# sjz5202/DisenLink

Hardware: AMD Instinct MI355X
Metric: edges/sec (aggregate+score) at K=8 d=64 (higher is better)
Workload: dtype f32; 1 GPU; squirrel_real (edge list of the parity fixture)(seed 0): N=5201, edge rows=217073, 85/5/10 split, E_sym=342129, scored train pairs P=1009603 (m=5), K=8, d=64, beta=0.5, t=1.0; forward route+aggregate+score_pairs; K=8, d=64, n_nodes=5201, E_sym=342129, P=1009603

## Files before the change

### disenlink_amd/_lib.py

```python
from __future__ import annotations

import ctypes as C
import os

PKG = os.path.dirname(os.path.abspath(__file__))
LIB_PATH = os.path.join(PKG, "libdisenlink_hip.so")


class DlCsrPlan(C.Structure):
    _fields_ = [
        ("n_rows", C.c_int32), ("row_offset", C.c_int32), ("n_total", C.c_int32), ("n_entries", C.c_int32),
        ("rowptr", C.c_void_p), ("col", C.c_void_p),
        ("seg_len", C.c_int32), ("n_seg", C.c_int32),
        ("seg_row", C.c_void_p), ("seg_beg", C.c_void_p), ("seg_end", C.c_void_p), ("seg_slot", C.c_void_p),
        ("n_slices", C.c_int32), ("slice_max_seg", C.c_int32), ("slice_seg0", C.c_void_p),
        ("n_multi", C.c_int32), ("n_slots", C.c_int32), ("multi_row", C.c_void_p), ("multi_slot0", C.c_void_p),
        ("slot_multi", C.c_void_p), ("unit_count", C.c_void_p),
    ]


class DlGraph(C.Structure):
    _fields_ = [("csr", DlCsrPlan), ("route", DlCsrPlan), ("rev", C.c_void_p), ("route_mirror", C.c_int32)]


class DlPairHub(C.Structure):
    _fields_ = [("n_blocks", C.c_int32), ("block_row", C.c_void_p),
                ("n_items", C.c_int32), ("n_slices", C.c_int32), ("slice_max_item", C.c_int32),
                ("slice_item0", C.c_void_p), ("item_block", C.c_void_p), ("item_step", C.c_void_p),
                ("n_steps", C.c_int32), ("step_v", C.c_void_p), ("step_u", C.c_void_p), ("step_q", C.c_void_p),
                ("step_q2", C.c_void_p), ("n_entries", C.c_int32),
                ("rest", DlCsrPlan), ("rest_pair", C.c_void_p), ("rest_pair2", C.c_void_p)]


class DlPairIncidence(C.Structure):
    _fields_ = [("csr", DlCsrPlan), ("inc_pair", C.c_void_p), ("n_pairs", C.c_int32), ("entry_yw", C.c_void_p),
                ("inc_pair2", C.c_void_p), ("n_second", C.c_int32), ("hub", C.POINTER(DlPairHub))]


class DlHostCsr(C.Structure):
    _fields_ = [("n_nodes", C.c_int32), ("n_entries", C.c_int32), ("rowptr", C.POINTER(C.c_int32)),
                ("col", C.POINTER(C.c_int32)), ("rev", C.POINTER(C.c_int32))]


class DlHostPlan(C.Structure):
    _fields_ = [(n, C.c_int32) for n in ("seg_len", "n_seg", "n_slices", "slice_max_seg", "n_multi", "n_slots")] + \
               [(n, C.POINTER(C.c_int32)) for n in ("seg_row", "seg_beg", "seg_end", "seg_slot", "slice_seg0",
# ... 301 lines not shown
```

### disenlink_amd/csrc/dl_api.hip

```cpp
#include <stdarg.h>
#include <string.h>
#include "dl_common.h"
#include "dl_kernels.h"

namespace dl {

static thread_local char g_err[512] = "";
static int g_force_generic = 0;

void set_error(const char* fmt, ...) {
    va_list ap;
    va_start(ap, fmt);
    vsnprintf(g_err, sizeof(g_err), fmt, ap);
    va_end(ap);
}

int check_launch(const char* what) {
    hipError_t e = hipGetLastError();
    if (e != hipSuccess) {
        set_error("%s: %s", what, hipGetErrorString(e));
        return DL_E_LAUNCH;
    }
    return DL_OK;
}
// ... 202 lines not shown
    if (int rc = check_dtype(c, K, d, dtype)) return rc;
    DL_REQUIRE(t != 0.0f, "temperature is 0");
    if (c->n_rows == 0) return DL_OK;
    DL_REQUIRE(Z && s, "Z or s is NULL");
    if (c->n_entries > 0) DL_REQUIRE(p && a, "p or a is NULL");
    if (use_fast(c, K, d, dtype)) {
        Workspace w;
        if (int rc = check_workspace(c, K, d, ws, ws_bytes, &w)) return rc;
        const dl_csr_plan* rp = &g->route;
        const bool have = has_seg_plan(rp) && rp->n_rows == c->n_rows && rp->n_total == c->n_total &&
                          rp->row_offset == c->row_offset && rp->rowptr == c->rowptr && rp->col == c->col;
        const bool mirror = have && g->route_mirror != 0;
        if (mirror)
            DL_REQUIRE((g->rev != nullptr || c->n_entries == 0) && c->row_offset == 0 && c->n_rows == c->n_total,
                       "route_mirror needs rev and an unsharded plan");
        return fast_route_fwd(c, have ? rp : nullptr, mirror, g->rev, Z, K, d, dtype, t, p, a, s, w.vec_part,
                              (hipStream_t)stream);
    }
    return generic_route_fwd(c, (const float*)Z, K, d, t, p, a, s, (hipStream_t)stream);
}

int dl_aggregate_fwd(const dl_graph* g, const void* Z, int K, int d, dl_dtype dtype, float beta, const uint8_t* p,
                     const float* a, const float* s, void* H, void* ws, size_t ws_bytes, void* stream) {
    DL_REQUIRE(g != nullptr, "graph is NULL");
    const dl_csr_plan* c = &g->csr;
    if (int rc = check_plan(c, "graph")) return rc;
    if (int rc = check_shape(K, d)) return rc;
    if (int rc = check_dtype(c, K, d, dtype)) return rc;
    if (c->n_rows == 0) return DL_OK;
    DL_REQUIRE(Z && s && H, "Z, s or H is NULL");
    if (c->n_entries > 0) DL_REQUIRE(p && a, "p or a is NULL");
// ... 878 lines not shown
```

### disenlink_amd/csrc/dl_config.h

```cpp
#pragma once

namespace dl {

struct Config {
    int stream_rows;
    bool fwd_group_kernel;
    bool fwd_hub;
    int auc_target;
    bool project_fp32_mfma;
    int fwd_groups;
    long long fwd_block_rows;
    long long bwd_block_bytes;
    int bwd_target;
    int inkernel_combine;
    int rank_slices;
    int mine_tiles;
    int sparse_seg;
};

const Config& config();
void config_reload();

}
```

### disenlink_amd/csrc/dl_config.hip

```cpp
#include <stdlib.h>
#include <algorithm>
#include <mutex>
#include "dl_config.h"
#include "disenlink_hip.h"

namespace dl {
namespace {

Config g_config;
std::once_flag g_once;

bool flag(const char* name) {
    const char* e = getenv(name);
    return e != nullptr && e[0] != '\0' && !(e[0] == '0' && e[1] == '\0');
}
long long number(const char* name) {
    const char* e = getenv(name);
    return e != nullptr && e[0] != '\0' ? atoll(e) : 0;
}

void read_environment() {
    Config c;
    const char* sr = getenv("DL_STREAM_ROWS");
    c.stream_rows = (sr == nullptr || sr[0] == '\0') ? -1 : (sr[0] == '1' ? 1 : 0);
    c.fwd_group_kernel = flag("DL_FWD_GROUP_KERNEL");
    const char* fh = getenv("DL_FWD_HUB");
    c.fwd_hub = !(fh != nullptr && fh[0] == '0' && fh[1] == '\0');
    c.auc_target = (int)std::max(0LL, number("DL_AUC_TARGET"));
    c.project_fp32_mfma = getenv("DL_PROJECT_FP32_MFMA") != nullptr;
    c.fwd_groups = (int)std::max(0LL, number("DL_FWD_GROUPS"));
    c.fwd_block_rows = std::max(0LL, number("DL_FWD_BLOCK_ROWS"));
    c.bwd_block_bytes = std::max(0LL, number("DL_BWD_BLOCK_BYTES"));
    c.bwd_target = (int)std::max(0LL, number("DL_BWD_TARGET"));
    const char* ic = getenv("DL_INKERNEL_COMBINE");
    c.inkernel_combine = (ic == nullptr || ic[0] == '\0') ? 1 : std::max(0, std::min(2, atoi(ic)));
    c.rank_slices = (int)std::max(0LL, number("DL_RANK_SLICES"));
    c.mine_tiles = (int)std::max(0LL, std::min(1LL << 20, number("DL_MINE_TILES")));
    c.sparse_seg = (int)std::max(0LL, std::min(1LL << 20, number("DL_SPARSE_SEG")));
    g_config = c;
}

}
// ... 15 lines not shown
```

### disenlink_amd/csrc/dl_fast.h

```cpp
#pragma once
#include <stdlib.h>
#include <type_traits>
#include "dl_common.h"
#include "dl_kernels.h"

namespace dl {
namespace fast {

typedef unsigned short bf16_t;

template <int VEC>
struct Chunk {
    float v[VEC];
};

__device__ __forceinline__ float bf16_to_f32(unsigned int hi16) { return __uint_as_float(hi16 << 16); }
__device__ __forceinline__ unsigned int f32_to_bf16(float f) {
    unsigned int u = __float_as_uint(f);
    if ((u & 0x7fffffffu) > 0x7f800000u) return (u >> 16) | 0x40u;
    return (u + 0x7fffu + ((u >> 16) & 1u)) >> 16;
}

template <typename T>
struct Tab;
// ... 139 lines not shown
typedef float v2f __attribute__((ext_vector_type(2)));
__device__ __forceinline__ float dot4_packed(const float4& a, const float4& b) {
    const v2f a0 = {a.x, a.y}, a1 = {a.z, a.w}, b0 = {b.x, b.y}, b1 = {b.z, b.w};
    const v2f p = __builtin_elementwise_fma(a1, b1, a0 * b0);
    return p.x + p.y;
}

template <typename V>
__device__ __forceinline__ const __attribute__((address_space(1))) V* uniform_row(const void* table, size_t byte_off) {
    const __attribute__((address_space(1))) char* row =
        reinterpret_cast<const __attribute__((address_space(1))) char*>((const __attribute__((address_space(1))) void*)table) + byte_off;
    asm volatile("" : "+s"(row));
    return reinterpret_cast<const __attribute__((address_space(1))) V*>(row);
}
__device__ __forceinline__ float4 as_float4(dl_vf4 v) { return make_float4(v.x, v.y, v.z, v.w); }

template <int K, int D, int VEC>
__device__ __forceinline__ void stage_row(float* dst, const Chunk<VEC> (&acc)[K], int c) {
#pragma unroll
    for (int kk = 0; kk < K; ++kk) store_f32<VEC>(dst + kk * D + c * VEC, acc[kk]);
}

template <int K, int D, typename T, int NROWS, bool NO_GROUP_ROWS = false>
struct Stage {
    using GE = Geo<K, D, T>;
    static constexpr int VEC = GE::VEC, G = GE::G;
    static constexpr int NG = DL_WAVE / G;
    static constexpr int ROWF = NROWS * GE::ROW;
    static constexpr bool GROUPS_IN_LDS = !NO_GROUP_ROWS && NROWS == 2 && (size_t)WAVES_PER_BLOCK * NG * ROWF * sizeof(float) <= 64 * 1024;
    static constexpr int SG = GROUPS_IN_LDS ? NG : 1;
// ... 198 lines not shown
```

### disenlink_amd/csrc/dl_kernels.h

```cpp
#pragma once
#include <hip/hip_runtime.h>
#include "disenlink_hip.h"

namespace dl {

int generic_route_fwd(const dl_csr_plan* c, const float* Z, int K, int d, float t, uint8_t* p, float* a, float* s,
                      hipStream_t st);
int generic_aggregate_fwd(const dl_csr_plan* c, const float* Z, int K, int d, float beta, const uint8_t* p,
                          const float* a, const float* s, float* H, hipStream_t st);
int generic_score_pairs_fwd(const float* Z, const float* H, int K, int d, float t, const int32_t* pu,
                            const int32_t* pv, int P, float* prob, hipStream_t st);
int generic_score_pairs_bwd(const dl_pair_incidence* inc, const float* Z, const float* H, int K, int d, float t,
                            const float* prob, const float* g_prob, float* dZ, float* dH, hipStream_t st);
int generic_bwd_phase1(const dl_csr_plan* c, const float* Z, int K, int d, float beta, const uint8_t* p,
                       const float* a, const float* s, const float* dH, float* dw, float* dwr, float* ds,
                       hipStream_t st);
int generic_bwd_phase2(const dl_csr_plan* c, const float* Z, int K, int d, float beta, float t, const uint8_t* p,
                       const float* a, const float* s, const float* dH, const float* dw, const float* dwr,
                       const float* ds, const float* dz_in, const float* scale, float* dZ, hipStream_t st);

bool fast_supported(int K, int d, int dtype);
int fast_route_fwd(const dl_csr_plan* g, const dl_csr_plan* route, bool mirror, const int32_t* rev, const void* Z,
                   int K, int d, int dtype, float t, uint8_t* p, float* a, float* s, float* s_part, hipStream_t st);
int fast_aggregate_fwd(const dl_csr_plan* g, const void* Z, int K, int d, int dtype, float beta, const uint8_t* p,
                       const float* a, const float* s, void* H, float* h_part, hipStream_t st);
int fast_bwd_phase1(const dl_csr_plan* g, const void* Z, int K, int d, int dtype, float beta, const uint8_t* p,
                    const float* a, const float* s, const float* dH, float* dw, float* dwr, float* ds,
                    float* ds_part, hipStream_t st);
int fast_bwd_phase2(const dl_csr_plan* g, const void* Z, int K, int d, int dtype, float beta, float t,
                    const uint8_t* p, const float* a, const float* s, const float* dH, const float* dw,
                    const float* dwr, const float* ds, const float* dz_in, const float* scale, float* dZ, float* dz_part, hipStream_t st);
int fast_score_pairs_fwd(const dl_pair_incidence* by_u, const void* Z, const void* H, int K, int d, int dtype,
                         float t, float* prob, float* coef, hipStream_t st);
int fast_score_pairs_train(const dl_pair_incidence* inc, const void* Z, const void* H, int K, int d, int dtype, float t,
                           const float* y, const float* w, float* prob, float* dZ, float* dH, float* part, hipStream_t st);
int fast_score_pairs_bwd(const dl_pair_incidence* inc, const void* Z, const void* H, int K, int d, int dtype,
                         float t, const float* prob, const float* g_prob, const float* coef, float* dZ, float* dH,
                         float* part, hipStream_t st);
// ... 150 lines not shown
```

### disenlink_amd/csrc/dl_route.hip

```cpp
#include "dl_fast.h"

namespace dl {
namespace fast {

template <int K, int D, typename T, bool MIRROR>
__global__ __launch_bounds__(BLOCK, (K <= 8 && sizeof(T) == 4) ? 8 : (K <= 10 ? 6 : (K <= 16 ? 4 : 1))) void route_seg_kernel(dl_csr_plan g, const int32_t* __restrict__ rev,
                                                          const T* __restrict__ Z, float t,
                                                          uint8_t* __restrict__ p, float* __restrict__ a) {
    using GE = Geo<K, D, T>;
    using FL = typename GE::FL;
    constexpr int VEC = GE::VEC, G = GE::G, EPW = GE::EPW, KP = FL::KP, VPL = FL::VPL;
    const WaveSeg ws = load_wave_seg(g);
    if (!ws.active) return;
    const SegInfo si = ws.si;
    const int lane = lane_id();
    const int c = lane % G, grp = lane / G;
    const int kb = FL::factor_base(c);

    Chunk<VEC> zi[K];
#pragma unroll
    for (int k = 0; k < K; ++k) zi[k] = Tab<T>::load(Z + (size_t)si.grow * GE::ROW + k * D + c * VEC);

    int my_col = si.grow, my_rev = 0;
    if (si.beg + lane < si.end) {
// ... 15 lines not shown
        int win = 255;
#pragma unroll
        for (int i = 0; i < VPL; ++i) {
            const float al = ex[i] / S;
            if (kb + i < K && (win == 255 || beats(al, best))) { best = al; win = kb + i; }
        }
        group_argmax_first<G>(best, win);
        if (MIRROR) {
            const int r = entry_scalar<EPW>(my_rev, base - si.beg, grp);
            if (live && c == 0) { p[e] = (uint8_t)win; a[e] = best; }
            if (live && c == 1 % G && r != e) { p[r] = (uint8_t)win; a[r] = best; }
        } else {
            if (live && c == 0) { p[e] = (uint8_t)win; a[e] = best; }
        }
    }
}

constexpr int ROWSUM_SUB = 4;
constexpr int ROWSUM_POS_PER_BLOCK = BLOCK / ROWSUM_SUB;

template <int CTRL>
__device__ __forceinline__ float dpp_move(float v) {
    return __int_as_float(__builtin_amdgcn_update_dpp(0, __float_as_int(v), CTRL, 0xF, 0xF, true));
}
template <int CTRL>
__device__ __forceinline__ int dpp_move_i(int v) {
    return __builtin_amdgcn_update_dpp(-1, v, CTRL, 0xF, 0xF, false);
}

template <int KP>
// ... 107 lines not shown
    else if (K <= 8) hipLaunchKernelGGL(s_rowsum_thread_kernel<8>, grid, block, 0, st, *g, K, p, a, s, reg);
    else if (K <= 16) hipLaunchKernelGGL(s_rowsum_thread_kernel<16>, grid, block, 0, st, *g, K, p, a, s, reg);
    else hipLaunchKernelGGL(s_rowsum_thread_kernel<32>, grid, block, 0, st, *g, K, p, a, s, reg);
}

void launch_vec_combine(const dl_csr_plan* g, int K, const float* part, int mode, const float* s_raw,
                        float* out, hipStream_t st) {
    if (g->n_multi <= 0) return;
    hipLaunchKernelGGL(vec_combine_kernel, dim3(wave_blocks(g->n_multi)), dim3(BLOCK), 0, st, *g, K, pow2_at_least(K),
                       part, mode, s_raw, out);
}

template <int K, int D, typename T>
struct RouteOps {
    static int route_fwd(const dl_csr_plan* g, const dl_csr_plan* route, bool mirror, const int32_t* rev,
                         const void* Z, float t, uint8_t* p, float* a, float* s, float* s_part, hipStream_t st) {
        const dl_csr_plan* rp = route ? route : g;
        if (mirror)
            hipLaunchKernelGGL((route_seg_kernel<K, D, T, true>), dim3(seg_blocks(rp)), dim3(BLOCK), 0, st, *rp, rev,
                               (const T*)Z, t, p, a);
        else
            hipLaunchKernelGGL((route_seg_kernel<K, D, T, false>), dim3(seg_blocks(rp)), dim3(BLOCK), 0, st, *rp, rev,
                               (const T*)Z, t, p, a);
        (void)s_part;
        launch_s_rowsum(g, K, p, a, s, st);
        return check_launch("route_fwd(fast)");
    }
};

}

bool fast_supported(int K, int d, int dtype) {
#define X(KK, DD) if (K == KK && d == DD) return true;
    if (dtype == DL_F32) { DL_FAST_SHAPES_F32(X) }
    if (dtype == DL_BF16) { DL_FAST_SHAPES_BF16(X) }
#undef X
    return false;
}

int fast_route_fwd(const dl_csr_plan* g, const dl_csr_plan* route, bool mirror, const int32_t* rev, const void* Z,
                   int K, int d, int dtype, float t, uint8_t* p, float* a, float* s, float* s_part, hipStream_t st) {
#define X_F32(KK, DD) \
    if (K == KK && d == DD) return fast::RouteOps<KK, DD, float>::route_fwd(g, route, mirror, rev, Z, t, p, a, s, s_part, st);
#define X_BF16(KK, DD)      \
    if (K == KK && d == DD) \
        return fast::RouteOps<KK, DD, fast::bf16_t>::route_fwd(g, route, mirror, rev, Z, t, p, a, s, s_part, st);
    DL_DISPATCH(X)
#undef X_F32
#undef X_BF16
}

}
```

### disenlink_amd/csrc/dl_score.hip

```cpp
#include "dl_fast.h"
#include "dl_score_bwd.h"

namespace dl {
namespace fast {

template <int K, int D, typename T, bool COEF>
__global__ __launch_bounds__(BLOCK, K <= 8 ? 4 : 1) void score_fwd_seg_kernel(dl_csr_plan g, const int32_t* __restrict__ pair_id,
                                                              const int32_t* __restrict__ pair_id2,
                                                              const T* __restrict__ Z, const T* __restrict__ H,
                                                              float t, float* __restrict__ prob,
                                                              float* __restrict__ coef_e,
                                                              float* __restrict__ coef_q) {
    using GE = Geo<K, D, T>;
    constexpr int VEC = GE::VEC, G = GE::G, EPW = GE::EPW, ROW = GE::ROW;
    constexpr int KB = K > 8 ? 8 : K;
    using FLB = FactorLanes<G, KB>;
    constexpr int KBP = FLB::KP;
    __shared__ __attribute__((aligned(16))) float urow[WAVES_PER_BLOCK][2 * ROW];
    const WaveSeg ws = load_wave_seg(g);
    const SegInfo si = ws.si;
    const int wave = ws.wave, lane = lane_id();
    const bool active = ws.active;
    if (active) stage_u_rows<K, D, T>(urow[wave], Z, H, (size_t)si.grow);
    __syncthreads();
// ... 145 lines not shown
                if (i < 8) coef_e[(size_t)qq * K + k] = ex;
                else coef_q[(size_t)qq * K + k] = ttv;
                if (FOLD && qq2 >= 0) {
                    if (i < 8) coef_e[(size_t)qq2 * K + k] = ex;
                    else coef_q[(size_t)qq2 * K + k] = ttv;
                }
            }
        }
    };
    const int nfull = len / U;
    for (int step = 0; step < nfull; ++step) do_step(step, std::false_type{}, U);
    if (len % U != 0) do_step(nfull, std::true_type{}, len % U);
}

namespace hub {
constexpr int WAVES = 8, THREADS = WAVES * DL_WAVE;

typedef int dl_vi4 __attribute__((ext_vector_type(4)));
__device__ __forceinline__ dl_vi4 plan_words(const int32_t* a, int idx) {
    const auto* g = (const __attribute__((address_space(1))) int32_t*)a;
    return reinterpret_cast<const __attribute__((address_space(4))) dl_vi4*>((const __attribute__((address_space(4))) int32_t*)g)[idx];
}

struct StepWords {
    dl_vi4 v, u, q, p;
};

__device__ __forceinline__ void transposed_reduce16_masked(float* v, int c) {
    float a[8], b[4];
    asm volatile("s_nop 1\n\t"
                 "v_add_f32_dpp %0, %8, %8 row_ror:8 row_mask:0xf bank_mask:0x3\n\t"
                 "v_add_f32_dpp %1, %9, %9 row_ror:8 row_mask:0xf bank_mask:0x3\n\t"
                 "v_add_f32_dpp %2, %10, %10 row_ror:8 row_mask:0xf bank_mask:0x3\n\t"
                 "v_add_f32_dpp %3, %11, %11 row_ror:8 row_mask:0xf bank_mask:0x3\n\t"
                 "v_add_f32_dpp %4, %12, %12 row_ror:8 row_mask:0xf bank_mask:0x3\n\t"
                 "v_add_f32_dpp %5, %13, %13 row_ror:8 row_mask:0xf bank_mask:0x3\n\t"
                 "v_add_f32_dpp %6, %14, %14 row_ror:8 row_mask:0xf bank_mask:0x3\n\t"
// ... 452 lines not shown
```

### disenlink_amd/graph.py

```python
from __future__ import annotations

import os
import ctypes as C
from dataclasses import dataclass, field

import torch

from . import _lib

DEFAULT_SEG_LEN = int(os.environ.get("DL_SEG_LEN", "32"))
DEFAULT_ROUTE_SEG_LEN = int(os.environ.get("DL_ROUTE_SEG_LEN", "0"))


def route_seg_len(n_entries: int) -> int:
    if DEFAULT_ROUTE_SEG_LEN:
        return DEFAULT_ROUTE_SEG_LEN
    return 16 if n_entries >= 16 * 4096 else 8
DEFAULT_INC_SEG_LEN = 64
DEFAULT_RUN_LEN = 64
DEFAULT_SLICES = 8
UNIT_SEGS = 4
L2_BYTES_PER_XCD = 4 << 20


# ... 259 lines not shown
    def c_value(self) -> _lib.DlCsrPlan:
        return _lib.DlCsrPlan(
            self.n_rows, self.row_offset, self.n_total, self.n_entries, self.rowptr.data_ptr(), self.col.data_ptr(),
            self.seg_len, self.n_seg, self.seg_row.data_ptr(), self.seg_beg.data_ptr(), self.seg_end.data_ptr(),
            self.seg_slot.data_ptr(), self.n_slices, self.slice_max_seg, self.slice_seg0.data_ptr(),
            int(self.multi_row.numel()), self.n_slots, self.multi_row.data_ptr(), self.multi_slot0.data_ptr(),
            self.slot_multi.data_ptr(), self.unit_count.data_ptr())


@dataclass
class Graph(_PlanOwner):
    plan: CsrPlan
    rev: torch.Tensor | None = None
    route: CsrPlan | None = None
    route_mirror: bool = False
    _struct: _lib.DlGraph | None = field(default=None, repr=False)
    _ws_need: dict = field(default_factory=dict, repr=False)

    def __post_init__(self):
        _assign_handle(self)

    n_nodes = property(lambda self: self.plan.n_total)
    n_rows = property(lambda self: self.plan.n_rows)
    row_offset = property(lambda self: self.plan.row_offset)
    n_edges = property(lambda self: self.plan.n_entries)
    n_seg = property(lambda self: self.plan.n_seg)
    rowptr = property(lambda self: self.plan.rowptr)
    col = property(lambda self: self.plan.col)
    device = property(lambda self: self.plan.device)

    @staticmethod
    def from_edge_rows(src: torch.Tensor, dst: torch.Tensor, n_nodes: int, symmetrise: bool = True,
                       seg_len: int = DEFAULT_SEG_LEN, row_range: tuple[int, int] | None = None,
                       row_bytes: int = 2048) -> "Graph":
        if n_nodes < 0 or n_nodes >= 2 ** 31:
            raise ValueError(f"n_nodes={n_nodes} out of int32 range")
        src = src.reshape(-1).to(torch.int64)
        dst = dst.reshape(-1).to(torch.int64)
        if src.numel() != dst.numel():
            raise ValueError("src and dst differ in length")
        if src.numel() and (int(src.min()) < 0 or int(dst.min()) < 0 or
                            int(src.max()) >= n_nodes or int(dst.max()) >= n_nodes):
            raise ValueError("edge endpoint outside [0, n_nodes)")
        if symmetrise:
            src, dst = torch.cat([src, dst]), torch.cat([dst, src])
        key = torch.unique(src * n_nodes + dst)
        if key.numel() >= 2 ** 31:
            raise ValueError("more than 2^31-1 edges")
        r = torch.div(key, n_nodes, rounding_mode="floor")
# ... 8 lines not shown
        if not (0 <= lo <= hi <= n_nodes):
            raise ValueError("row_range outside [0, n_nodes]")
        counts = torch.bincount(r, minlength=n_nodes) if key.numel() else torch.zeros(n_nodes, dtype=torch.int64,
                                                                                      device=key.device)
        full_ptr = torch.zeros(n_nodes + 1, dtype=torch.int64, device=key.device)
        full_ptr[1:] = torch.cumsum(counts, dim=0)
        e0, e1 = int(full_ptr[lo]), int(full_ptr[hi])
        by_len = length_order(n_nodes, row_bytes)
        plan = CsrPlan.build(full_ptr[lo:hi + 1] - e0, c[e0:e1], n_nodes, row_offset=lo, seg_len=seg_len, by_length=by_len)
        mirror = row_range is None
        lc, lr = c[e0:e1], r[e0:e1] - lo
        route = CsrPlan.build(full_ptr[lo:hi + 1] - e0, lc, n_nodes, row_offset=lo,
                              seg_len=min(seg_len, route_seg_len((e1 - e0 + 1) // 2 if mirror else e1 - e0)), n_slices=1,
                              keep=(lc >= lr + lo) if mirror else None, unit_segs=1, by_length=by_len)
        route.rowptr, route.col = plan.rowptr, plan.col
        return Graph(plan, _i32(rev) if mirror else None, route, mirror)

    @staticmethod
    def from_dense(adj: torch.Tensor, seg_len: int = DEFAULT_SEG_LEN, row_bytes: int = 2048) -> "Graph":
        if adj.dim() != 2 or adj.shape[0] != adj.shape[1]:
            raise ValueError("adj must be square")
        if adj.layout != torch.strided:
            coo = adj.to_sparse_coo().coalesce()
            val, idx = coo.values(), coo.indices()
            if bool(((val != 0) & (val != 1)).any()):
                raise ValueError("adj must hold 0 / 1 entries (the reference's layer multiplies by it, model.py:62)")
            keep = val != 0
            return Graph.from_edge_rows(idx[0][keep], idx[1][keep], adj.shape[0], symmetrise=False, seg_len=seg_len,
                                        row_bytes=row_bytes)
        nz = torch.nonzero(adj)
        if nz.shape[0] and bool((adj[nz[:, 0], nz[:, 1]] != 1).any()):
            raise ValueError("adj must hold 0 / 1 entries (the reference's layer multiplies by it, model.py:62)")
        return Graph.from_edge_rows(nz[:, 0], nz[:, 1], adj.shape[0], symmetrise=False, seg_len=seg_len,
                                    row_bytes=row_bytes)

    def to(self, device) -> "Graph":
        plan = self.plan.to(device)
        route = None if self.route is None else self.route.to(device)
        if route is not None:
            route.rowptr, route.col = plan.rowptr, plan.col
        return Graph(plan, None if self.rev is None else self.rev.to(device), route, self.route_mirror)

    def c_struct(self):
        if self._struct is None:
            rp = self.route.c_value() if self.route is not None else _lib.DlCsrPlan()
            self._struct = _lib.DlGraph(self.plan.c_value(), rp, self.rev.data_ptr() if self.rev is not None else None,
                                        1 if self.route_mirror else 0)
        return C.byref(self._struct)

    def c_plan(self):
        self.c_struct()
        return C.byref(self._struct.csr)


def mirror_partners(pu: torch.Tensor, pv: torch.Tensor, n_nodes: int) -> torch.Tensor:
    P, dev = pu.numel(), pu.device
    second = torch.full((P,), -1, dtype=torch.int64, device=dev)
    if P == 0:
        return second
    lo_, hi_ = torch.minimum(pu, pv), torch.maximum(pu, pv)
    okey = pu * n_nodes + pv
    order = torch.argsort(okey, stable=True)
# ... 67 lines not shown
    n_entries: int
    rest: CsrPlan | None
    rest_pair: torch.Tensor | None
    rest_pair2: torch.Tensor | None
    _struct: _lib.DlPairHub | None = field(default=None, repr=False)

    @property
    def n_steps(self) -> int:
        return int(self.step_v.shape[0])

    @property
    def n_gathered(self) -> int:
        return int((self.step_v >= 0).sum())

    @staticmethod
    def build(row, col, pair, pair2, n_nodes: int, n_rows: int, n_slices: int, bounds, rest_csr) -> "HubPlan":
        dev = row.device
        ar = lambda n: torch.arange(n, device=dev)
        excl = lambda x: torch.cumsum(x, 0) - x
        rank, order, n_live = hub_rank(row, n_nodes)
        T = max(0, min(int(n_rows), n_live))
        nb = (T + HUB_W - 1) // HUB_W
        block_row = torch.full((nb * HUB_W,), -1, dtype=torch.int64, device=dev)
        block_row[:T] = order[:T]
        in_hub = rank[row] < T
        hrow, v, q = row[in_hub], col[in_hub], pair[in_hub]
        q2 = None if pair2 is None else pair2[in_hub]
        E = int(v.numel())
        blk = torch.div(rank[hrow], HUB_W, rounding_mode="floor")
        ul = rank[hrow] - blk * HUB_W
        sl = torch.bucketize(v, bounds.to(dev), right=True) if n_slices > 1 else torch.zeros_like(v)
# ... 5 lines not shown
        gnew = torch.ones(E, dtype=torch.bool, device=dev)
        gnew[1:] = key[1:] != key[:-1]
        gfirst = torch.nonzero(gnew).reshape(-1)
        g_of = torch.cumsum(gnew, 0) - 1
        G = int(gfirst.numel())
        c = torch.bincount(g_of, minlength=G)
        g_bs = torch.div(key[gfirst], n_nodes, rounding_mode="floor")
        nC, rem = torch.div(c, 4, rounding_mode="floor"), c % 4
        hasB, hasA = (rem >= 2).long(), ((rem == 1) | (rem == 3)).long()
        gath = nC + hasB + hasA
        bs_new = torch.ones(G, dtype=torch.bool, device=dev)
        bs_new[1:] = g_bs[1:] != g_bs[:-1]
        bs_first = torch.nonzero(bs_new).reshape(-1)
        bs_of = torch.cumsum(bs_new, 0) - 1
        cum = excl(gath)
        part = torch.div(cum - cum[bs_first][bs_of], HUB_ITEM_ROWS, rounding_mode="floor")
        inew = bs_new.clone()
        inew[1:] |= part[1:] != part[:-1]
        ifirst = torch.nonzero(inew).reshape(-1)
        i_of = torch.cumsum(inew, 0) - 1
        I = int(ifirst.numel())
        within = lambda x: excl(x) - excl(x)[ifirst][i_of]
        cC, cB, cA = within(nC), within(hasB), within(hasA)
        tot = lambda x: torch.zeros(I, dtype=torch.int64, device=dev).index_add_(0, i_of, x)
        nC_i, nB_i, nA_i = tot(nC), (tot(hasB) + 1) // 2, (tot(hasA) + 3) // 4
        n_i = nA_i + nB_i + nC_i
        i_blk = torch.div(g_bs[ifirst], n_slices, rounding_mode="floor")
        i_sl = g_bs[ifirst] - i_blk * n_slices
        big = int(n_i.max()) + 1 if I else 1
        iperm = torch.argsort(((i_sl % n_streams) * (n_slices + 1) + i_sl) * big + (big - 1 - n_i), stable=True)
        ipos = torch.empty_like(iperm)
# ... 30 lines not shown
        rest = rest_pair = rest_pair2 = None
        if int((~in_hub).sum()):
            got = rest_csr(~in_hub)
            rest, rest_pair = got[0], got[1]
            rest_pair2 = got[2] if len(got) > 2 else None
        item_block = torch.empty(I, dtype=torch.int64, device=dev)
        item_block[ipos] = i_blk
        item_slice = torch.empty(I, dtype=torch.int64, device=dev)
        item_slice[ipos] = i_sl
        item_step_s = torch.empty_like(item_step)
        item_step_s[ipos] = item_step
        return HubPlan(T, nb, _i32(block_row), I, n_streams, int(per_stream.max()) if I else 0, _i32(slice_item0),
                       _i32(item_block), _i32(item_slice), _i32(item_step_s), _i32(step_v), _i32(step_u), _i32(step_q),
                       None if step_q2 is None else _i32(step_q2), E, rest, rest_pair, rest_pair2)

    def check(self) -> None:
        if self.n_items == 0:
            return
        dev = self.step_v.device
        st = self.item_step.long()
        lens = torch.stack([st[:, 1] - st[:, 0], st[:, 2] - st[:, 1], st[:, 3] - st[:, 2]], dim=1).reshape(-1)
        ends = torch.cumsum(lens, 0)
        ok = bool((lens >= 0).all()) and int(ends[-1]) == self.n_steps and bool((st[1:, 0] == st[:-1, 3]).all()) \
            and int(st[0, 0]) == 0
        if ok:
            nv = torch.repeat_interleave(torch.tensor([4, 2, 1], device=dev).repeat(self.n_items), lens)
            last = torch.zeros(self.n_steps, dtype=torch.bool, device=dev)
            last[(ends - 1)[lens > 0]] = True
            used = torch.arange(4, device=dev)[None, :] < nv[:, None]
            live = (self.step_v >= 0) & used
# ... 2 lines not shown
                and not bool((live[:, 1:] & ~live[:, :-1]).any())
        if not ok:
            raise ValueError("hub plan: dead partner rows may only close the last step of an item's A list and B list "
                             "(dl_pair_hub, disenlink_hip.h)")

    def c_value(self) -> _lib.DlPairHub:
        if self._struct is None:
            self.check()
            ptr = lambda t: None if t is None else t.data_ptr()
            self._struct = _lib.DlPairHub(
                self.n_blocks, ptr(self.block_row), self.n_items, self.n_slices, self.slice_max_item, ptr(self.slice_item0),
                ptr(self.item_block), ptr(self.item_step), self.n_steps, ptr(self.step_v), ptr(self.step_u),
                ptr(self.step_q), ptr(self.step_q2), self.n_entries,
                self.rest.c_value() if self.rest is not None else _lib.DlCsrPlan(), ptr(self.rest_pair), ptr(self.rest_pair2))
        return self._struct


@dataclass
class PairList(_PlanOwner):
    n_nodes: int
    pu: torch.Tensor
    pv: torch.Tensor
    by_u: CsrPlan
    by_u_pair: torch.Tensor
    inc: CsrPlan
    inc_pair: torch.Tensor
    fwd: CsrPlan | None = None
    fwd_pair: torch.Tensor | None = None
    fwd_pair2: torch.Tensor | None = None
    hub: HubPlan | None = None
# ... 129 lines not shown
```

### include/disenlink_hip.h

```cpp
#ifndef DISENLINK_HIP_H
#define DISENLINK_HIP_H

#include <stddef.h>
#include <stdint.h>

#ifdef __cplusplus
extern "C" {
#endif

#define DL_OK            0
#define DL_E_ARG        -1
#define DL_E_LAUNCH     -2
#define DL_E_WORKSPACE  -3

#define DL_MAX_FACTORS  64

typedef enum dl_dtype { DL_F32 = 0, DL_BF16 = 1 } dl_dtype;

#define DL_UNIT_SEGS 4
typedef struct dl_csr_plan {
    int32_t n_rows;
    int32_t row_offset;
    int32_t n_total;
    int32_t n_entries;
// ... 9 lines not shown
    int32_t slice_max_seg;
    const int32_t* slice_seg0;
    int32_t n_multi;
    int32_t n_slots;
    const int32_t* multi_row;
    const int32_t* multi_slot0;
    const int32_t* slot_multi;
    int32_t* unit_count;
} dl_csr_plan;

typedef struct dl_graph {
    dl_csr_plan csr;
    dl_csr_plan route;
    const int32_t* rev;
    int32_t route_mirror;
} dl_graph;

typedef struct dl_pair_incidence {
    dl_csr_plan csr;
    const int32_t* inc_pair;
    int32_t n_pairs;
    const float* entry_yw;
    const int32_t* inc_pair2;
    int32_t n_second;
    const struct dl_pair_hub* hub;
} dl_pair_incidence;

#define DL_HUB_W 16
typedef struct dl_pair_hub {
    int32_t n_blocks;
// ... 357 lines not shown
```

Baseline: 8.508 billion edges/s.

## Route edges through hub-blocked plan staging owner rows in LDS

Adds a hub-style routing kernel for f32, d=64, K=4/8. Upper-triangle edges are grouped by their higher-degree endpoint, and those owner rows are staged in shared memory so partner rows stream through once per block. Softmax and argmax are computed per edge and written to both mirrored slots. The aim is to cut repeated global gathers of Z in the route step, at the cost of a host-side plan build and extra complexity. The path is on by default when the graph is built unsharded with a mirror.

```diff
diff --git a/disenlink_amd/_lib.py b/disenlink_amd/_lib.py
--- a/disenlink_amd/_lib.py
+++ b/disenlink_amd/_lib.py
@@ -19,10 +19,6 @@
     ]
 
 
-class DlGraph(C.Structure):
-    _fields_ = [("csr", DlCsrPlan), ("route", DlCsrPlan), ("rev", C.c_void_p), ("route_mirror", C.c_int32)]
-
-
 class DlPairHub(C.Structure):
     _fields_ = [("n_blocks", C.c_int32), ("block_row", C.c_void_p),
                 ("n_items", C.c_int32), ("n_slices", C.c_int32), ("slice_max_item", C.c_int32),
@@ -30,6 +26,11 @@
                 ("n_steps", C.c_int32), ("step_v", C.c_void_p), ("step_u", C.c_void_p), ("step_q", C.c_void_p),
                 ("step_q2", C.c_void_p), ("n_entries", C.c_int32),
                 ("rest", DlCsrPlan), ("rest_pair", C.c_void_p), ("rest_pair2", C.c_void_p)]
+
+
+class DlGraph(C.Structure):
+    _fields_ = [("csr", DlCsrPlan), ("route", DlCsrPlan), ("rev", C.c_void_p), ("route_mirror", C.c_int32),
+                ("route_hub", C.POINTER(DlPairHub))]
 
 
 class DlPairIncidence(C.Structure):
diff --git a/disenlink_amd/csrc/dl_api.hip b/disenlink_amd/csrc/dl_api.hip
--- a/disenlink_amd/csrc/dl_api.hip
+++ b/disenlink_amd/csrc/dl_api.hip
@@ -240,7 +240,20 @@
         if (mirror)
             DL_REQUIRE((g->rev != nullptr || c->n_entries == 0) && c->row_offset == 0 && c->n_rows == c->n_total,
                        "route_mirror needs rev and an unsharded plan");
-        return fast_route_fwd(c, have ? rp : nullptr, mirror, g->rev, Z, K, d, dtype, t, p, a, s, w.vec_part,
+        const dl_pair_hub* hp = nullptr;
+        if (g->route_hub != nullptr && mirror && config().route_hub && fast_route_hub_supported(K, d, dtype) &&
+            g->route_hub->n_items > 0) {
+            hp = g->route_hub;
+            DL_REQUIRE(hp->rest.n_entries == 0 && 2LL * hp->n_entries >= c->n_entries && hp->n_entries <= c->n_entries,
+                       "route_hub must hold each of the graph's entries with col >= row (%d entries in all) and no residual plan: "
+                       "it holds %d + %d", c->n_entries, hp->n_entries, hp->rest.n_entries);
+            DL_REQUIRE(hp->n_slices >= 1 && hp->slice_max_item >= 1 && hp->n_blocks >= 1 && hp->n_steps >= 1, "route_hub: empty grid");
+            DL_REQUIRE(hp->block_row && hp->slice_item0 && hp->item_block && hp->item_step && hp->step_v && hp->step_u &&
+                       hp->step_q && hp->step_q2, "route_hub: NULL array");
+            DL_REQUIRE((((uintptr_t)hp->step_v | (uintptr_t)hp->step_u | (uintptr_t)hp->step_q | (uintptr_t)hp->step_q2) & 15) == 0,
+                       "route_hub: step_v, step_u, step_q and step_q2 must be 16-byte aligned");
+        }
+        return fast_route_fwd(c, have ? rp : nullptr, mirror, g->rev, hp, Z, K, d, dtype, t, p, a, s, w.vec_part,
                               (hipStream_t)stream);
     }
     return generic_route_fwd(c, (const float*)Z, K, d, t, p, a, s, (hipStream_t)stream);
diff --git a/disenlink_amd/csrc/dl_config.h b/disenlink_amd/csrc/dl_config.h
--- a/disenlink_amd/csrc/dl_config.h
+++ b/disenlink_amd/csrc/dl_config.h
@@ -6,6 +6,7 @@
     int stream_rows;
     bool fwd_group_kernel;
     bool fwd_hub;
+    bool route_hub;
     int auc_target;
     bool project_fp32_mfma;
     int fwd_groups;
diff --git a/disenlink_amd/csrc/dl_config.hip b/disenlink_amd/csrc/dl_config.hip
--- a/disenlink_amd/csrc/dl_config.hip
+++ b/disenlink_amd/csrc/dl_config.hip
@@ -26,6 +26,8 @@
     c.fwd_group_kernel = flag("DL_FWD_GROUP_KERNEL");
     const char* fh = getenv("DL_FWD_HUB");
     c.fwd_hub = !(fh != nullptr && fh[0] == '0' && fh[1] == '\0');
+    const char* rh = getenv("DL_ROUTE_HUB");
+    c.route_hub = !(rh != nullptr && rh[0] == '0' && rh[1] == '\0');
     c.auc_target = (int)std::max(0LL, number("DL_AUC_TARGET"));
     c.project_fp32_mfma = getenv("DL_PROJECT_FP32_MFMA") != nullptr;
     c.fwd_groups = (int)std::max(0LL, number("DL_FWD_GROUPS"));
diff --git a/disenlink_amd/csrc/dl_fast.h b/disenlink_amd/csrc/dl_fast.h
--- a/disenlink_amd/csrc/dl_fast.h
+++ b/disenlink_amd/csrc/dl_fast.h
@@ -177,6 +177,16 @@
     return reinterpret_cast<const __attribute__((address_space(1))) V*>(row);
 }
 __device__ __forceinline__ float4 as_float4(dl_vf4 v) { return make_float4(v.x, v.y, v.z, v.w); }
+
+namespace hub {
+constexpr int WAVES = 8, THREADS = WAVES * DL_WAVE;
+
+typedef int dl_vi4 __attribute__((ext_vector_type(4)));
+__device__ __forceinline__ dl_vi4 plan_words(const int32_t* a, int idx) {
+    const auto* g = (const __attribute__((address_space(1))) int32_t*)a;
+    return reinterpret_cast<const __attribute__((address_space(4))) dl_vi4*>((const __attribute__((address_space(4))) int32_t*)g)[idx];
+}
+}
 
 template <int K, int D, int VEC>
 __device__ __forceinline__ void stage_row(float* dst, const Chunk<VEC> (&acc)[K], int c) {
diff --git a/disenlink_amd/csrc/dl_kernels.h b/disenlink_amd/csrc/dl_kernels.h
--- a/disenlink_amd/csrc/dl_kernels.h
+++ b/disenlink_amd/csrc/dl_kernels.h
@@ -20,8 +20,10 @@
                        const float* ds, const float* dz_in, const float* scale, float* dZ, hipStream_t st);
 
 bool fast_supported(int K, int d, int dtype);
-int fast_route_fwd(const dl_csr_plan* g, const dl_csr_plan* route, bool mirror, const int32_t* rev, const void* Z,
-                   int K, int d, int dtype, float t, uint8_t* p, float* a, float* s, float* s_part, hipStream_t st);
+int fast_route_fwd(const dl_csr_plan* g, const dl_csr_plan* route, bool mirror, const int32_t* rev, const dl_pair_hub* hub,
+                   const void* Z, int K, int d, int dtype, float t, uint8_t* p, float* a, float* s, float* s_part,
+                   hipStream_t st);
+bool fast_route_hub_supported(int K, int d, int dtype);
 int fast_aggregate_fwd(const dl_csr_plan* g, const void* Z, int K, int d, int dtype, float beta, const uint8_t* p,
                        const float* a, const float* s, void* H, float* h_part, hipStream_t st);
 int fast_bwd_phase1(const dl_csr_plan* g, const void* Z, int K, int d, int dtype, float beta, const uint8_t* p,
diff --git a/disenlink_amd/csrc/dl_route.hip b/disenlink_amd/csrc/dl_route.hip
--- a/disenlink_amd/csrc/dl_route.hip
+++ b/disenlink_amd/csrc/dl_route.hip
@@ -53,6 +53,166 @@
             if (live && c == 0) { p[e] = (uint8_t)win; a[e] = best; }
         }
     }
+}
+
+namespace hub {
+template <int K, int D>
+struct RouteGeo {
+    static constexpr bool ok = D == 64 && (K == 4 || K == 8);
+    static constexpr int NJ = K * D / 256;
+    static constexpr int NVAL = 4 * NJ;
+    static constexpr int SH = K == 8 ? 1 : 2;
+};
+constexpr int ROUTE_MAXW = 6;
+
+struct RouteWords {
+    dl_vi4 v, u;
+};
+
+__device__ __forceinline__ float dot4_chain(const float4& x, const float4& y) {
+    float r = x.x * y.x;
+    r = fmaf(x.y, y.y, r);
+    r = fmaf(x.z, y.z, r);
+    return fmaf(x.w, y.w, r);
+}
+
+template <int OFF>
+__device__ __forceinline__ void argmax_xor(float& best, int& win) {
+    const float ob = xor_lane<OFF>(best);
+    const int ow = xor_lane_i<OFF>(win);
+    const bool o_nan = ob != ob, b_nan = best != best;
+    const bool o_beats = (ob > best) | (o_nan & !b_nan), b_beats = (best > ob) | (b_nan & !o_nan);
+    const bool take = o_beats | (!b_beats & (ow < win));
+    best = take ? ob : best;
+    win = take ? ow : win;
+}
+
+template <int K, int D, bool T1>
+__global__ __launch_bounds__(THREADS) __attribute__((amdgpu_waves_per_eu(4, ROUTE_MAXW))) void route_seg_kernel(
+    dl_pair_hub h, const float* __restrict__ Z, float t, uint8_t* __restrict__ p, float* __restrict__ a) {
+    using RG = RouteGeo<K, D>;
+    constexpr int NJ = RG::NJ, NVAL = RG::NVAL, SH = RG::SH, ROW = K * D, R4 = ROW / 4;
+    static_assert(RG::ok, "one DPP row of 16 lanes per factor slice, one or two chunks");
+    static_assert(DL_HUB_W == 2 * WAVES, "every wave stages two rows of the block");
+    __shared__ __attribute__((aligned(16))) float4 urow[DL_HUB_W * R4];
+    int it = (int)blockIdx.x;
+    if (h.n_slices > 1) {
+        const int x = blockIdx.x % h.n_slices;
+        it = h.slice_item0[x] + (int)(blockIdx.x / h.n_slices);
+        if (it >= h.slice_item0[x + 1]) return;
+    } else if (it >= h.n_items) {
+        return;
+    }
+    const int wave = wave_index(), lane = lane_id();
+    const int i = lane & 15, r = lane >> 4;
+    const int blk = h.item_block[it];
+    const int s_a = h.item_step[4 * it], s_b = h.item_step[4 * it + 1], s_c = h.item_step[4 * it + 2],
+              s_end = h.item_step[4 * it + 3];
+    auto fetch = [&](const int step) {
+        const int s = __builtin_amdgcn_readfirstlane(step);
+        RouteWords w;
+        w.v = plan_words(h.step_v, s), w.u = plan_words(h.step_u, s);
+        return w;
+    };
+    constexpr int NB = 1 << SH;
+    const int e_me = (i >> SH) & 3;
+    const int k_me = 4 * (i >> (SH + 2)) + r;
+    const int b_me = i & (NB - 1);
+    const bool writer = (i >> (SH + 2)) == 0 && r < 2;
+    float sg = 0.0f;
+    int nb = 0, dst = -1;
+    const int32_t* const my_q = r == 0 ? h.step_q : h.step_q2;
+    auto open = [&](const int s0) {
+        const int sb = s0 + WAVES * b_me;
+        dst = -1;
+        if (writer && sb < s_end) dst = my_q[4 * sb + e_me];
+    };
+    auto flush = [&]() {
+        const float ex = expf(T1 ? sg : sg / t);
+        float S = ex;
+        if constexpr (NJ == 2) S = add_xor<8>(S);
+        S = add_xor<16>(add_xor<32>(S));
+        float best = ex / S;
+        int win = k_me;
+        if constexpr (NJ == 2) argmax_xor<8>(best, win);
+        argmax_xor<32>(best, win);
+        argmax_xor<16>(best, win);
+        if (dst >= 0) {
+            p[dst] = (uint8_t)win;
+            a[dst] = best;
+        }
+    };
+    auto tick = [&](const int step) {
+        if (nb == NB) {
+            flush();
+            nb = 0;
+            open(step + WAVES);
+        }
+    };
+    auto do_step = [&](const RouteWords& w, auto shape, auto last) {
+        constexpr int NV = decltype(shape)::value;
+        constexpr bool LAST = decltype(last)::value;
+        const int sv[4] = {w.v.x, w.v.y, w.v.z, w.v.w}, su[4] = {w.u.x, w.u.y, w.u.z, w.u.w};
+        float4 zv[NV][NJ];
+#pragma unroll
+        for (int n = 0; n < NV; ++n) {
+            if (!LAST || sv[n] >= 0) {
+                const auto* zr = uniform_row<dl_vf4>(Z, (size_t)(unsigned)sv[n] * ROW * sizeof(float));
+#pragma unroll
+                for (int j = 0; j < NJ; ++j) zv[n][j] = as_float4(zr[(unsigned)(lane + j * 64)]);
+            } else {
+#pragma unroll
+                for (int j = 0; j < NJ; ++j) zv[n][j] = make_float4(0.0f, 0.0f, 0.0f, 0.0f);
+            }
+        }
+        float val[NVAL];
+#pragma unroll
+        for (int j = 0; j < NJ; ++j) {
+            float4 u4[4];
+#pragma unroll
+            for (int e = 0; e < 4; ++e) u4[e] = urow[(su[e] & (DL_HUB_W - 1)) * R4 + j * 64 + lane];
+            __builtin_amdgcn_sched_barrier(0);
+#pragma unroll
+            for (int e = 0; e < 4; ++e) val[j * 4 + e] = dot4_chain(u4[e], zv[e * NV / 4][j]);
+            __builtin_amdgcn_sched_barrier(0);
+        }
+        TransposedReduce<NVAL, 8>::run(val, i);
+        sg = b_me == nb ? val[0] : sg;
+        ++nb;
+    };
+    using FULL = std::false_type;
+    using LAST = std::true_type;
+    constexpr std::integral_constant<int, 4> SHAPE_A{};
+    constexpr std::integral_constant<int, 2> SHAPE_B{};
+    constexpr std::integral_constant<int, 1> SHAPE_C{};
+    int s = s_a + wave;
+    RouteWords nxt = {};
+    if (s < s_end) nxt = fetch(s);
+    open(s);
+#pragma unroll
+    for (int rr = 0; rr < 2; ++rr) {
+        const int ul = 2 * wave + rr;
+        const int row = h.block_row[blk * DL_HUB_W + ul];
+#pragma unroll
+        for (int j = 0; j < NJ; ++j) {
+            float4 z4 = make_float4(0.0f, 0.0f, 0.0f, 0.0f);
+            if (row >= 0) z4 = *reinterpret_cast<const float4*>(Z + (size_t)row * ROW + (j * 64 + lane) * 4);
+            urow[ul * R4 + j * 64 + lane] = z4;
+        }
+    }
+    __syncthreads();
+    auto take = [&](const int step) {
+        const RouteWords w = nxt;
+        if (step + WAVES < s_end) nxt = fetch(step + WAVES);
+        return w;
+    };
+    for (; s < s_b - 1; s += WAVES) do_step(take(s), SHAPE_A, FULL{}), tick(s);
+    if (s == s_b - 1) do_step(take(s), SHAPE_A, LAST{}), tick(s), s += WAVES;
+    for (; s < s_c - 1; s += WAVES) do_step(take(s), SHAPE_B, FULL{}), tick(s);
+    if (s == s_c - 1) do_step(take(s), SHAPE_B, LAST{}), tick(s), s += WAVES;
+    for (; s < s_end; s += WAVES) do_step(take(s), SHAPE_C, FULL{}), tick(s);
+    if (nb > 0) flush();
+}
 }
 
 constexpr int ROWSUM_SUB = 4;
@@ -190,7 +350,19 @@
 template <int K, int D, typename T>
 struct RouteOps {
     static int route_fwd(const dl_csr_plan* g, const dl_csr_plan* route, bool mirror, const int32_t* rev,
-                         const void* Z, float t, uint8_t* p, float* a, float* s, float* s_part, hipStream_t st) {
+                         const dl_pair_hub* hp, const void* Z, float t, uint8_t* p, float* a, float* s, float* s_part,
+                         hipStream_t st) {
+        if constexpr (std::is_same<T, float>::value && hub::RouteGeo<K, D>::ok) {
+            if (hp != nullptr) {
+                const dim3 grid((unsigned)hp->n_slices * (unsigned)hp->slice_max_item), block(hub::THREADS);
+                if (t == 1.0f)
+                    hipLaunchKernelGGL((hub::route_seg_kernel<K, D, true>), grid, block, 0, st, *hp, (const float*)Z, t, p, a);
+                else
+                    hipLaunchKernelGGL((hub::route_seg_kernel<K, D, false>), grid, block, 0, st, *hp, (const float*)Z, t, p, a);
+                launch_s_rowsum(g, K, p, a, s, st);
+                return check_launch("route_fwd(fast, hub blocks)");
+            }
+        }
         const dl_csr_plan* rp = route ? route : g;
         if (mirror)
             hipLaunchKernelGGL((route_seg_kernel<K, D, T, true>), dim3(seg_blocks(rp)), dim3(BLOCK), 0, st, *rp, rev,
@@ -214,13 +386,16 @@
     return false;
 }
 
-int fast_route_fwd(const dl_csr_plan* g, const dl_csr_plan* route, bool mirror, const int32_t* rev, const void* Z,
-                   int K, int d, int dtype, float t, uint8_t* p, float* a, float* s, float* s_part, hipStream_t st) {
+bool fast_route_hub_supported(int K, int d, int dtype) { return dtype == DL_F32 && d == 64 && (K == 4 || K == 8); }
+
+int fast_route_fwd(const dl_csr_plan* g, const dl_csr_plan* route, bool mirror, const int32_t* rev, const dl_pair_hub* hub,
+                   const void* Z, int K, int d, int dtype, float t, uint8_t* p, float* a, float* s, float* s_part,
+                   hipStream_t st) {
 #define X_F32(KK, DD) \
-    if (K == KK && d == DD) return fast::RouteOps<KK, DD, float>::route_fwd(g, route, mirror, rev, Z, t, p, a, s, s_part, st);
+    if (K == KK && d == DD) return fast::RouteOps<KK, DD, float>::route_fwd(g, route, mirror, rev, hub, Z, t, p, a, s, s_part, st);
 #define X_BF16(KK, DD)      \
     if (K == KK && d == DD) \
-        return fast::RouteOps<KK, DD, fast::bf16_t>::route_fwd(g, route, mirror, rev, Z, t, p, a, s, s_part, st);
+        return fast::RouteOps<KK, DD, fast::bf16_t>::route_fwd(g, route, mirror, rev, hub, Z, t, p, a, s, s_part, st);
     DL_DISPATCH(X)
 #undef X_F32
 #undef X_BF16
diff --git a/disenlink_amd/csrc/dl_score.hip b/disenlink_amd/csrc/dl_score.hip
--- a/disenlink_amd/csrc/dl_score.hip
+++ b/disenlink_amd/csrc/dl_score.hip
@@ -183,13 +183,6 @@
 }
 
 namespace hub {
-constexpr int WAVES = 8, THREADS = WAVES * DL_WAVE;
-
-typedef int dl_vi4 __attribute__((ext_vector_type(4)));
-__device__ __forceinline__ dl_vi4 plan_words(const int32_t* a, int idx) {
-    const auto* g = (const __attribute__((address_space(1))) int32_t*)a;
-    return reinterpret_cast<const __attribute__((address_space(4))) dl_vi4*>((const __attribute__((address_space(4))) int32_t*)g)[idx];
-}
 
 struct StepWords {
     dl_vi4 v, u, q, p;
diff --git a/disenlink_amd/graph.py b/disenlink_amd/graph.py
--- a/disenlink_amd/graph.py
+++ b/disenlink_amd/graph.py
@@ -297,6 +297,7 @@
     rev: torch.Tensor | None = None
     route: CsrPlan | None = None
     route_mirror: bool = False
+    route_hub: HubPlan | None = None
     _struct: _lib.DlGraph | None = field(default=None, repr=False)
     _ws_need: dict = field(default_factory=dict, repr=False)
 
@@ -315,7 +316,7 @@
     @staticmethod
     def from_edge_rows(src: torch.Tensor, dst: torch.Tensor, n_nodes: int, symmetrise: bool = True,
                        seg_len: int = DEFAULT_SEG_LEN, row_range: tuple[int, int] | None = None,
-                       row_bytes: int = 2048) -> "Graph":
+                       row_bytes: int = 2048, route_hub: bool | None = None) -> "Graph":
         if n_nodes < 0 or n_nodes >= 2 ** 31:
             raise ValueError(f"n_nodes={n_nodes} out of int32 range")
         src = src.reshape(-1).to(torch.int64)
@@ -354,10 +355,14 @@
                               seg_len=min(seg_len, route_seg_len((e1 - e0 + 1) // 2 if mirror else e1 - e0)), n_slices=1,
                               keep=(lc >= lr + lo) if mirror else None, unit_segs=1, by_length=by_len)
         route.rowptr, route.col = plan.rowptr, plan.col
-        return Graph(plan, _i32(rev) if mirror else None, route, mirror)
+        if route_hub and not mirror:
+            raise ValueError("a routing hub plan needs the unsharded graph (row_range=None)")
+        hub = route_hub_plan(lr, lc, rev, n_nodes, force=bool(route_hub)) if mirror and route_hub is not False else None
+        return Graph(plan, _i32(rev) if mirror else None, route, mirror, hub)
 
     @staticmethod
-    def from_dense(adj: torch.Tensor, seg_len: int = DEFAULT_SEG_LEN, row_bytes: int = 2048) -> "Graph":
+    def from_dense(adj: torch.Tensor, seg_len: int = DEFAULT_SEG_LEN, row_bytes: int = 2048,
+                   route_hub: bool | None = None) -> "Graph":
         if adj.dim() != 2 or adj.shape[0] != adj.shape[1]:
             raise ValueError("adj must be square")
         if adj.layout != torch.strided:
@@ -367,25 +372,34 @@
                 raise ValueError("adj must hold 0 / 1 entries (the reference's layer multiplies by it, model.py:62)")
             keep = val != 0
             return Graph.from_edge_rows(idx[0][keep], idx[1][keep], adj.shape[0], symmetrise=False, seg_len=seg_len,
-                                        row_bytes=row_bytes)
+                                        row_bytes=row_bytes, route_hub=route_hub)
         nz = torch.nonzero(adj)
         if nz.shape[0] and bool((adj[nz[:, 0], nz[:, 1]] != 1).any()):
             raise ValueError("adj must hold 0 / 1 entries (the reference's layer multiplies by it, model.py:62)")
         return Graph.from_edge_rows(nz[:, 0], nz[:, 1], adj.shape[0], symmetrise=False, seg_len=seg_len,
-                                    row_bytes=row_bytes)
+                                    row_bytes=row_bytes, route_hub=route_hub)
 
     def to(self, device) -> "Graph":
         plan = self.plan.to(device)
         route = None if self.route is None else self.route.to(device)
         if route is not None:
             route.rowptr, route.col = plan.rowptr, plan.col
-        return Graph(plan, None if self.rev is None else self.rev.to(device), route, self.route_mirror)
+        return Graph(plan, None if self.rev is None else self.rev.to(device), route, self.route_mirror,
+                     None if self.route_hub is None else self.route_hub.to(device))
 
     def c_struct(self):
         if self._struct is None:
             rp = self.route.c_value() if self.route is not None else _lib.DlCsrPlan()
             self._struct = _lib.DlGraph(self.plan.c_value(), rp, self.rev.data_ptr() if self.rev is not None else None,
                                         1 if self.route_mirror else 0)
+            h = self.route_hub
+            if h is not None and h.n_items > 0:
+                row = torch.repeat_interleave(torch.arange(self.n_rows, device=self.device), (self.rowptr[1:] - self.rowptr[:-1]).long())
+                n_upper = int((self.col.long() >= row).sum())
+                if not self.route_mirror or h.rest is not None or h.step_q2 is None or h.n_entries != n_upper:
+                    raise ValueError(f"routing hub plan: needs a mirrored graph, no residual plan and each of the {n_upper} "
+                                     f"entries with col >= row as a slot (it holds {h.n_entries})")
+                self._struct.route_hub = C.pointer(h.c_value())
         return C.byref(self._struct)
 
     def c_plan(self):
@@ -483,7 +497,9 @@
         return int((self.step_v >= 0).sum())
 
     @staticmethod
-    def build(row, col, pair, pair2, n_nodes: int, n_rows: int, n_slices: int, bounds, rest_csr) -> "HubPlan":
+    def build(row, col, pair, pair2, n_nodes: int, n_rows: int, n_slices: int, bounds, rest_csr,
+              item_rows: int | None = None) -> "HubPlan":
+        item_rows = HUB_ITEM_ROWS if item_rows is None else int(item_rows)
         dev = row.device
         ar = lambda n: torch.arange(n, device=dev)
         excl = lambda x: torch.cumsum(x, 0) - x
@@ -519,7 +535,7 @@
         bs_first = torch.nonzero(bs_new).reshape(-1)
         bs_of = torch.cumsum(bs_new, 0) - 1
         cum = excl(gath)
-        part = torch.div(cum - cum[bs_first][bs_of], HUB_ITEM_ROWS, rounding_mode="floor")
+        part = torch.div(cum - cum[bs_first][bs_of], item_rows, rounding_mode="floor")
         inew = bs_new.clone()
         inew[1:] |= part[1:] != part[:-1]
         ifirst = torch.nonzero(inew).reshape(-1)
@@ -580,6 +596,13 @@
                        _i32(item_block), _i32(item_slice), _i32(item_step_s), _i32(step_v), _i32(step_u), _i32(step_q),
                        None if step_q2 is None else _i32(step_q2), E, rest, rest_pair, rest_pair2)
 
+    def to(self, device) -> "HubPlan":
+        mv = lambda t: None if t is None else t.to(device)
+        return HubPlan(self.n_rows, self.n_blocks, mv(self.block_row), self.n_items, self.n_slices, self.slice_max_item,
+                       mv(self.slice_item0), mv(self.item_block), mv(self.item_slice), mv(self.item_step), mv(self.step_v),
+                       mv(self.step_u), mv(self.step_q), mv(self.step_q2), self.n_entries, mv(self.rest),
+                       mv(self.rest_pair), mv(self.rest_pair2))
+
     def check(self) -> None:
         if self.n_items == 0:
             return
@@ -612,6 +635,28 @@
                 ptr(self.step_q), ptr(self.step_q2), self.n_entries,
                 self.rest.c_value() if self.rest is not None else _lib.DlCsrPlan(), ptr(self.rest_pair), ptr(self.rest_pair2))
         return self._struct
+
+
+ROUTE_HUB_ITEM_ROWS = 128
+ROUTE_HUB_SLICES = 4
+
+
+def route_hub_plan(row: torch.Tensor, col: torch.Tensor, rev: torch.Tensor, n_nodes: int, force: bool = False) -> HubPlan | None:
+    e = torch.nonzero(col >= row).reshape(-1)
+    if e.numel() == 0:
+        return None
+    r, c = row[e], col[e]
+    deg = torch.bincount(row, minlength=n_nodes)
+    swap = deg[c] > deg[r]
+    owner, partner = torch.where(swap, c, r), torch.where(swap, r, c)
+    e2 = rev[e]
+    e2 = torch.where(e2 == e, torch.full_like(e2, -1), e2)
+    T = int((torch.bincount(owner, minlength=n_nodes) > 0).sum()) if force else auto_hub_rows(owner, partner, n_nodes)
+    if T == 0:
+        return None
+    S = ROUTE_HUB_SLICES
+    bnd = slice_bounds(partner, S) if S > 1 else None
+    return HubPlan.build(owner, partner, e, e2, n_nodes, T, S, bnd, None, item_rows=ROUTE_HUB_ITEM_ROWS)
 
 
 @dataclass
diff --git a/include/disenlink_hip.h b/include/disenlink_hip.h
--- a/include/disenlink_hip.h
+++ b/include/disenlink_hip.h
@@ -47,6 +47,7 @@
     dl_csr_plan route;
     const int32_t* rev;
     int32_t route_mirror;
+    const struct dl_pair_hub* route_hub;
 } dl_graph;
 
 typedef struct dl_pair_incidence {
```

After: 8.792 billion edges/s, median of 6. +3.3%, better.
